# Elliotshui/ABRSimulator

Hardware: AMD Instinct MI355X
Metric: env_steps_per_sec (higher is better)
Workload: dtype f64

## Files before the change

abrsimulator_amd/_lib.py:

```python
import ctypes as C
import os
import subprocess

os.environ.setdefault("HIP_FORCE_DEV_KERNARG", "1")

import torch

_HERE = os.path.dirname(os.path.abspath(__file__))
CSRC = os.path.join(_HERE, "csrc")
DIAG_LIB_DIR = os.path.join(os.path.dirname(_HERE), "tools", "diag", "lib")


def resolve(name):
    if os.sep in name or os.path.isabs(name):
        return os.path.abspath(name)
    for d in (DIAG_LIB_DIR, CSRC):
        if os.path.exists(os.path.join(d, name)):
            return os.path.join(d, name)
    return os.path.join(DIAG_LIB_DIR, name)


SO_PATH = os.path.join(CSRC, "libabr_hip.so")
if os.environ.get("ABR_HIP_LIB"):
    SO_PATH = resolve(os.environ["ABR_HIP_LIB"])
# ... 171 lines not shown
    ("abr_env_step_policy_sampled", C.c_int, [_P, C.POINTER(Policy), C.POINTER(PolicySampling), C.c_int32, _P, _P, _P,
                                              _P, _P, _P, _P, _P]),
    ("abr_env_policy_select_ac", C.c_int, [_P, C.POINTER(Policy), C.POINTER(PolicySampling), C.POINTER(PolicyValue), _P, _P,
                                           _P, _P, _P, _P]),
    ("abr_env_step_policy_ac", C.c_int, [_P, C.POINTER(Policy), C.POINTER(PolicySampling), C.POINTER(PolicyValue),
                                         C.c_int32, _P, _P, _P, _P, _P, _P, _P, _P, _P, _P]),
    ("abr_policy_mx_weights_bytes", C.c_int, [C.POINTER(PolicyMx), C.c_int32, C.POINTER(C.c_size_t)]),
    ("abr_env_policy_select_mx", C.c_int, [_P, C.POINTER(PolicyMx), C.POINTER(PolicySampling), C.POINTER(PolicyValue), _P,
                                           _P, _P, _P, _P, _P]),
    ("abr_env_step_policy_mx", C.c_int, [_P, C.POINTER(PolicyMx), C.POINTER(PolicySampling), C.POINTER(PolicyValue),
                                         C.c_int32, _P, _P, _P, _P, _P, _P, _P, _P, _P, _P]),
    ("abr_gae", C.c_int, [_P, _P, _P, _P, _P, C.c_int32, C.c_int64, C.c_float, C.c_float, _P, _P, _P]),
    ("abr_debug_chain", C.c_int, [C.c_int32, C.c_int32, _P, _P, _P, _P, C.c_int64, _P, _P, _P, _P]),
    ("abr_debug_selfcheck", C.c_int, [_P, _P, _P]),
    ("abr_debug_drain", C.c_int, [C.c_double, C.c_double, _P, _P, C.c_int64, _P, _P, _P, C.POINTER(C.c_int32), _P]),
    ("abr_mpc_objective_grid", C.c_int, [C.POINTER(MpcConfig), C.c_int32, C.c_int32, C.c_double,
                                         _P, _P, _P, _P, _P]),
]

_libs = {}


class AbrError(RuntimeError):
    pass


def build(force=False, target="libabr_hip.so"):
    subprocess.check_call(["make", "-C", CSRC, "-s"] + (["-B"] if force else []) + [target])
    return os.path.join(CSRC, target)

# ... 44 lines not shown
```

abrsimulator_amd/csrc/abr_env.hip:

```cpp
#include <hip/hip_runtime.h>

#include <climits>
#include <cmath>
#include <cstdarg>
#include <cstdio>
#include <cstdlib>
#include <cstring>
#include <new>
#include <type_traits>
#include <vector>

#include "abr_env.h"

#ifdef ABR_SPLIT_STAMPS
#include "abr_diag_stamps.h"
#else
#define ABR_STAMP(n)
#define ABR_STAMP_INIT()
#define ABR_STAMP_FLUSH()
#define ABR_WG_TIME(slot)
#define ABR_WG_WHERE(role)
#define K3_STAMP_DECL
#define K3_STAMP(n)
#define K3_STAMP_FLUSH()
// ... 50 lines not shown
    int32_t speed_rows;
    int32_t *pl_left, *play_id;
    double *pt_sum;
    const double *br_table;
    long long *sumk;
    int32_t *k, *chunk_id, *n_su, *n_rb, *n_play, *j, *tpos, *trace_id, *offset0;
    int32_t *last_action, *n_su_obs, *n_rb_obs, *episode_no;
    uint8_t *flags, *done;
    uint8_t *action_hist;
    double *bw_hist;
    double *ep_qoe_terms;
    double *var_run;
    uint32_t *selfcheck_out;
    uint64_t sentinel;
    abrx::SpeedRuleBlock speed_rule;
};
static_assert(offsetof(EnvParams, speed_rule) == ABR_RULE_KERNARG_OFFSET, "abr_lane_jump.h reads the rule at this offset");
static_assert(sizeof(EnvParams) == 880, "the parameter block: 592 bytes + 288 of the speed rule");
static_assert(sizeof(abrx::SpeedRule) == sizeof(abr_speed_rule) &&
              offsetof(abrx::SpeedRule, lat_thr) == offsetof(abr_speed_rule, lat_thr) &&
              offsetof(abrx::SpeedRule, buf_thr) == offsetof(abr_speed_rule, buf_thr) &&
              offsetof(abrx::SpeedRule, speed) == offsetof(abr_speed_rule, speed), "abr_speed_rule: one layout");

constexpr uint32_t kTagMagic = 0x57524241u;
constexpr uint32_t kLayoutRev = 1;
struct WorkspaceTag {
    uint32_t magic, abi_version, layout_rev, n_rates;
    int64_t n_lanes;
    int32_t video_length, max_ticks, n_intervals, reserved_;
    uint64_t total_bytes;
    double chunk_length, interval, speed;
    uint8_t pad_[256 - 72];
};
static_assert(sizeof(WorkspaceTag) == 256, "the tag is one 256-byte block");
static_assert(sizeof(abrx::EpisodeSampler) == sizeof(abr_episode_sampler) &&
              offsetof(abrx::EpisodeSampler, pool) == offsetof(abr_episode_sampler, pool) &&
              offsetof(abrx::EpisodeSampler, n_pool) == offsetof(abr_episode_sampler, n_pool) &&
              offsetof(abrx::EpisodeSampler, offset_span) == offsetof(abr_episode_sampler, offset_span),
              "abr_episode_sampler: one layout");
static_assert(sizeof(abrx::EpisodeLedger) == sizeof(abr_episode_ledger) &&
// ... 373 lines not shown
        if (MODE != 0) {
            for (int32_t t = step_idx; t < n_total; t++) {
                const int64_t o = (int64_t)t * p.n_lanes + i;
                if (reward_out) reward_out[o] = 0.0f;
                if (done_out) done_out[o] = done;
                if ((MODE == 2 || MODE == 4) && actions_out) actions_out[o] = -1;
                if (obs_out)
                    write_obs(s, p, i, obs_out + (int64_t)t * ABR_OBS_DIM * p.n_lanes, last_bw);
            }
        }
    }
}

using abrx::LaneJ;

__device__ inline abrx::Tables make_tables(const EnvParams &p, bool cascade = true) {
    abrx::Tables t;
    t.G = p.G; t.interval_tick = p.interval_tick; t.avail_tick = p.avail_tick;
    t.L = p.chunk_length; t.sd = p.sd; t.max_buffer = p.max_buffer;
    t.start_up_length = p.start_up_length; t.V = p.video_length; t.max_ticks = p.max_ticks;
    t.per_lane_speed = p.lane_speeds != nullptr;
    t.speed_rows = p.lane_speeds ? p.speed_rows : 0;
    t.speed_stride = p.n_lanes; t.speeds = p.lane_speeds;
    t.drain = p.drain;
    if (p.lane_speeds || !cascade) t.drain.n = 0;
#ifdef ABR_NO_DRAIN_CASCADE
    t.drain.n = 0;
#endif
    return t;
}

__device__ inline void lanej_load(LaneJ &s, const EnvParams &p, int64_t i) {
    s.buf = p.buf[i]; s.sumk = p.sumk[i];
    s.k = p.k[i]; s.chunk_id = p.chunk_id[i]; s.n_su = p.n_su[i]; s.n_rb = p.n_rb[i];
    s.n_play = p.n_play[i]; s.cur.j = p.j[i]; s.cur.tpos = p.tpos[i];
    s.last_action = p.last_action[i];
    const uint8_t f = p.flags[i];
    s.su = f & kFlagStartUp; s.be = f & kFlagBufEmpty; s.bf = f & kFlagBufFull;
    const int32_t c = s.chunk_id < p.video_length ? s.chunk_id : p.video_length;
    s.avail_k = p.avail_tick[c];
    if (p.lane_speeds) { s.sd = p.sd_lane[i]; s.pt = p.pt_lane[i]; } else { s.sd = p.sd; s.pt = 0.0; }
    s.lane = i; s.pl_left = 0; s.play_id = 0; s.pt_sum = 0.0;
    if (p.lane_speeds && p.speed_rows >= 2) { s.pl_left = p.pl_left[i]; s.play_id = p.play_id[i]; s.pt_sum = p.pt_sum[i]; }
// ... 45 lines not shown

#ifndef ABR_JUMP_WAVES
#define ABR_JUMP_WAVES 5
#endif
#define ABR_JUMP_BOUNDS(MODE, SAMPLE) __launch_bounds__(64, ((MODE) == 1 || (MODE) == 4 || (SAMPLE) ? 4 : ABR_JUMP_WAVES))
template <int MODE, bool SAMPLE = false, bool LEDGER = false>
__global__ ABR_JUMP_BOUNDS(MODE, SAMPLE || LEDGER) void env_jump_kernel(
    EnvParams p, const int32_t *__restrict__ actions, const int32_t *__restrict__ trace_id_in,
    const int32_t *__restrict__ offset_in, const uint8_t *__restrict__ lane_mask,
    float *__restrict__ obs_out, float *__restrict__ reward_out, uint8_t *__restrict__ done_out,
    int32_t *__restrict__ actions_out, int32_t n_steps, uint64_t seed, abrx::RuleParams rule,
    abrx::EpisodeSampler smp, abrx::EpisodeLedger led) {
    const int64_t i = (int64_t)blockIdx.x * 64 + threadIdx.x;
    const bool in_range = i < p.n_lanes;
    const int32_t n_total = (MODE >= 2) ? n_steps : 1;
    const abrx::Tables tb = make_tables(p);
    LaneJ s;
    bool active = in_range, touched = in_range;
    uint8_t done = 0;
    int32_t n_su_obs = 0, n_rb_obs = 0, episode_no = 0, offset0 = 0;
    double last_bw = 0.0, hist_n = 0.0, hist_s = 0.0, var_run = 0.0;
    double g_su_obs = 0.0, g_rb_obs = 0.0;

    if (in_range) {
        if (MODE == 0) {
            if (lane_mask && !lane_mask[i]) { active = false; touched = false; }
            if (active) {
                int32_t t;
                if constexpr (SAMPLE) {
                    sampled_episode(p, smp, i, (p.flags[i] & kFlagArmed) ? p.episode_no[i] + 1 : 0, t, offset0);
                } else {
// ... 183 lines not shown
    out[ABR_F64_CHUNK_ID * n + i] = (double)p.chunk_id[i];
    out[ABR_F64_PLAY_ID * n + i] = sched ? (double)p.play_id[i] : (double)(p.n_play[i] / P);
    out[ABR_F64_LAST_BITRATE * n + i] = (double)p.last_action[i];
    out[ABR_F64_FLAGS * n + i] = (double)p.flags[i];
    out[ABR_F64_HIST_N * n + i] = p.hist_n[i];
    out[ABR_F64_HIST_SUM_INV * n + i] = p.hist_s[i];
    out[ABR_F64_TICK * n + i] = (double)p.k[i];
    out[ABR_F64_DOWNLOAD_TIME * n + i] = 0.0;
}

static size_t align_up(size_t x, size_t a) { return (x + a - 1) / a * a; }
static size_t mpc_scratch_bytes_max(size_t n_lanes) {
    return n_lanes * ((size_t)ABR_MAX_HORIZON * sizeof(double) + 2 * sizeof(int32_t));
}

struct Layout {
    size_t G, GP, interval_tick, avail_tick;
    size_t f64_state, i64_state, i32_state, u8_state, action_hist, bw_hist, ep_terms;
    size_t mpc_action, mpc_scratch;
    size_t tag;
    size_t total;
    int32_t max_ticks, n_intervals;
};

static double min_episode_ticks(const abr_env_config *c) {
    return ((double)c->video_length + 1.0) * ceil(c->chunk_length / kDt);
}
static double default_max_ticks(const abr_env_config *c) {
    double per_chunk = ceil(c->chunk_length / kDt);
    double mt = 32.0 * c->video_length * per_chunk;
    if (mt > 16.0e6) mt = 16.0e6;
    if (mt < 2.0 * min_episode_ticks(c)) mt = 2.0 * min_episode_ticks(c);
// ... 30 lines not shown
        return fail(ABR_E_INVALID, "max_ticks %g is below (video_length + 1) * ceil(chunk_length / dt) = %g: "
                    "every lane would end in ABR_DONE_TIMEOUT", mtd, min_episode_ticks(c));
    const int32_t mt = (int32_t)mtd;
    double n_iv = (double)mt * kDt / c->interval + 4.0;
    if (n_iv > 32.0e6)
        return fail(ABR_E_UNSUPPORTED, "interval %g s needs a %g-entry tick table", c->interval, n_iv);
    L->max_ticks = mt;
    L->n_intervals = (int32_t)n_iv;
    size_t o = 0;
    const size_t A = 256;
    size_t N = (size_t)n_lanes, V = (size_t)c->video_length;
    L->G = o; o = align_up(o + sizeof(double) * ((size_t)mt + 2), A);
    L->GP = o; o = align_up(o + sizeof(double) * ((size_t)mt + 2), A);
    L->interval_tick = o; o = align_up(o + sizeof(int32_t) * ((size_t)L->n_intervals + 8), A);
    L->avail_tick = o; o = align_up(o + sizeof(int32_t) * (V + 2), A);
    L->f64_state = o; o = align_up(o + sizeof(double) * 8 * N, A);
    L->i64_state = o; o = align_up(o + sizeof(long long) * 1 * N, A);
    L->i32_state = o; o = align_up(o + sizeof(int32_t) * 15 * N, A);
    L->u8_state = o; o = align_up(o + 2 * N, A);
    L->action_hist = o; o = align_up(o + V * N, A);
    L->bw_hist = o; o = align_up(o + sizeof(double) * V * N, A);
    L->ep_terms = o; o = align_up(o + sizeof(double) * 4 * N, A);
    L->mpc_action = o; o = align_up(o + sizeof(int32_t) * N, A);
    L->mpc_scratch = o; o = align_up(o + mpc_scratch_bytes_max(N), A);
    L->tag = o; o = align_up(o + sizeof(WorkspaceTag), A);
    L->total = o;
    return ABR_OK;
}

extern "C" int abr_env_workspace_bytes(const abr_env_config *cfg, int64_t n_lanes,
// ... 42 lines not shown
    EnvParams &p = e->p;
    p.n_rates = cfg->n_rates; p.video_length = cfg->video_length; p.max_ticks = mt;
    p.auto_reset = cfg->auto_reset; p.play_ticks_per_chunk = P; p.n_intervals = L.n_intervals;
    p.t_block = t_block; p.n_traces = n_traces;
    p.chunk_length = cfg->chunk_length; p.max_buffer = cfg->max_buffer;
    p.start_up_length = cfg->start_up_length;
    p.wr = cfg->rebuffer_weight; p.wv = cfg->variance_weight; p.ws = cfg->startup_weight;
    p.wl = cfg->latency_weight; p.sd = sd;
    for (int r = 0; r < ABR_MAX_RATES; r++) p.ladder[r] = cfg->ladder[r];
    p.n_lanes = n_lanes; p.lane_id_base = 0;
    char *w = (char *)workspace_dev;
    p.G = (const double *)(w + L.G); p.GP = (const double *)(w + L.GP);
    p.interval_tick = (const int32_t *)(w + L.interval_tick);
    p.avail_tick = (const int32_t *)(w + L.avail_tick);
    p.drain = abrx::make_drain_tab(sd, cfg->max_buffer + cfg->chunk_length);
    p.traces = traces_dev; p.trace_off = trace_off_dev; p.trace_len = trace_len_dev;
    const size_t N = (size_t)n_lanes;
    double *f = (double *)(w + L.f64_state);
    p.buf = f; p.last_bw = f + N; p.hist_n = f + 2 * N; p.hist_s = f + 3 * N;
    p.sd_lane = f + 4 * N; p.pt_lane = f + 5 * N; p.pt_sum = f + 6 * N; p.var_run = f + 7 * N; p.lane_speeds = nullptr;
    p.speed_rows = 1;
    p.speed_rule = abrx::SpeedRuleBlock{};
    p.sumk = (long long *)(w + L.i64_state);
    int32_t *q = (int32_t *)(w + L.i32_state);
    p.k = q; p.chunk_id = q + N; p.n_su = q + 2 * N; p.n_rb = q + 3 * N; p.n_play = q + 4 * N;
    p.j = q + 5 * N; p.tpos = q + 6 * N; p.trace_id = q + 7 * N; p.offset0 = q + 8 * N;
    p.last_action = q + 9 * N; p.n_su_obs = q + 10 * N; p.n_rb_obs = q + 11 * N;
    p.episode_no = q + 12 * N; p.pl_left = q + 13 * N; p.play_id = q + 14 * N;
    uint8_t *u = (uint8_t *)(w + L.u8_state);
    p.flags = u; p.done = u + N;
    p.action_hist = (uint8_t *)(w + L.action_hist);
    p.bw_hist = (double *)(w + L.bw_hist);
    p.ep_qoe_terms = (double *)(w + L.ep_terms);
    e->mpc_action = (int32_t *)(w + L.mpc_action);
    e->mpc_scratch = (void *)(w + L.mpc_scratch);

    hipStream_t st = (hipStream_t)stream;
    hipError_t he;
#define UP(dst, vec)                                                                           \
    he = hipMemcpyAsync((void *)(dst), (vec).data(), (vec).size() * sizeof((vec)[0]),          \
                        hipMemcpyHostToDevice, st);                                            \
    if (he != hipSuccess) { delete e; return fail(ABR_E_HIP, "table upload: %s", hipGetErrorString(he)); }
    UP(p.G, G) UP(p.GP, GP) UP(p.interval_tick, itick) UP(p.avail_tick, atick)
#undef UP
    he = hipMemsetAsync(w + L.f64_state, 0, L.total - L.f64_state, st);
    if (he == hipSuccess) he = hipMemsetAsync(p.done, ABR_DONE_EPISODE, N, st);
    {
        WorkspaceTag &tg = e->tag;
        memset(&tg, 0, sizeof(tg));
        tg.magic = kTagMagic; tg.abi_version = ABR_ABI_VERSION; tg.layout_rev = kLayoutRev; tg.n_rates = (uint32_t)cfg->n_rates;
        tg.n_lanes = n_lanes; tg.video_length = cfg->video_length; tg.max_ticks = mt; tg.n_intervals = L.n_intervals;
        tg.total_bytes = L.total; tg.chunk_length = cfg->chunk_length; tg.interval = cfg->interval; tg.speed = cfg->speed;
        e->tag_dev = w + L.tag;
        if (he == hipSuccess) he = hipMemcpyAsync(e->tag_dev, &tg, sizeof(tg), hipMemcpyHostToDevice, st);
    }
    if (he == hipSuccess) he = hipStreamSynchronize(st);
    if (he != hipSuccess) { delete e; return fail(ABR_E_HIP, "workspace init: %s", hipGetErrorString(he)); }
    *env_out = e;
// ... 2272 lines not shown

extern "C" int abr_debug_drain(double sd, double max_level, const double *x0_dev, const int32_t *n_dev, int64_t count,
                               double *x_out_dev, int32_t *a_out_dev, uint8_t *hit_out_dev, int32_t *stages_out,
                               void *stream) {
    if (!x0_dev || !n_dev || !x_out_dev || !a_out_dev || !hit_out_dev) return fail(ABR_E_INVALID, "NULL device pointer");
    if (count < 1) return fail(ABR_E_INVALID, "count must be >= 1");
    const abrx::DrainTab tab = abrx::make_drain_tab(sd, max_level);
    if (stages_out) *stages_out = tab.n;
    if (tab.n == 0) return fail(ABR_E_UNSUPPORTED, "no cascade for sd %g below %g: the kernels use the general chains", sd, max_level);
    hipLaunchKernelGGL(drain_debug_kernel, dim3((unsigned)((count + 63) / 64)), dim3(64), 0, (hipStream_t)stream, tab, sd,
                       x0_dev, n_dev, count, x_out_dev, a_out_dev, hit_out_dev);
    HIP_TRY(hipGetLastError());
    return ABR_OK;
}

__global__ void mpc_grid_kernel(int B, int H, int V, double L, double max_buffer, double wv,
                                double wr, int chunk, int prev, double buffer,
                                const double *__restrict__ pred, const double *__restrict__ br,
                                const double *__restrict__ sz, double *__restrict__ J_out,
                                int64_t total) {
    const int64_t f = (int64_t)blockIdx.x * blockDim.x + threadIdx.x;
    if (f >= total) return;
    int R[ABR_MAX_HORIZON + 1];
    {
        int64_t t = f;
        for (int i = H; i >= 1; i--) { R[i] = (int)(t % B); t /= B; }
        R[0] = prev < 0 ? prev + B : prev;
    }
    double q = 0.0, v = 0.0, rb = 0.0, buf = buffer;
    for (int i = 0; i < H; i++) {
// ... 44 lines not shown
```

abrsimulator_amd/csrc/abr_env_roles.h:

```cpp
#ifndef ABR_ENV_ROLES_H
#define ABR_ENV_ROLES_H


#ifndef ABR_SPLIT3_CASCADE
#define ABR_SPLIT3_CASCADE 0
#endif
#ifndef ABR_PRIO_D
#define ABR_PRIO_D 2
#endif
#ifndef ABR_PRIO_P
#define ABR_PRIO_P 1
#endif
#ifndef ABR_PRIO_S
#define ABR_PRIO_S 0
#endif

struct SplitMail {
    double dl[2][64];
    int32_t n_dl[2][64], k_start[2][64], step[2][64], action[2][64], avail_next[2][64], flags[2][64];
    int32_t fb_step[2][64], fb_k[2][64], fb_chunk[2][64], fb_episode[2][64], fb_alive[2][64];
    double fb_buf[2][64];
    int32_t fb_pf[2][64];
    int32_t any_alive[2];
};
// ... 273 lines not shown
    v.episode_no = 0; v.b_step = 0; v.b_alive = false; v.was_done = true;
}

__device__ __forceinline__ void role_p3_begin(PVars &v, const EnvParams &p) {
    const int64_t i = (int64_t)blockIdx.x * 64 + (threadIdx.x & 63);
    player_clear(v, p);
    if (i < p.n_lanes) {
        v.was_done = p.done[i] != 0;
        lanej_load(v.s, p, i);
        v.episode_no = p.episode_no[i];
        v.b_alive = !v.was_done;
    }
    ABR_STAMP_INIT();
}

template <int MODE, class M2>
__device__ __forceinline__ void role_p3_pre(PVars &v, const EnvParams &p, SplitMail &m, M2 &m2,
                                            int32_t n_total, int32_t t, int cb2) {
    const int l = threadIdx.x & 63;
    const int cb = t & 1, pb = (t + 1) & 1;
    const abrx::Tables tb = make_tables(p, ABR_SPLIT3_CASCADE != 0);
    const bool speeds = p.lane_speeds != nullptr;
    LaneJ &s = v.s;
    int32_t meta = 0;
    ABR_STAMP(8);
    if (v.b_alive && v.b_step < n_total && t >= 1) {
        int32_t fl = m.flags[pb][l];
        int32_t r_step = m.step[pb][l], r_k = m.k_start[pb][l], r_a = m.action[pb][l], r_ndl = m.n_dl[pb][l],
                r_avail = m.avail_next[pb][l];
        double r_dl = m.dl[pb][l];
        asm volatile("" : "+v"(fl), "+v"(r_step), "+v"(r_k), "+v"(r_a), "+v"(r_ndl), "+v"(r_avail), "+v"(r_dl));
        if ((fl & kRecValid) && r_step == v.b_step && r_k == s.k) {
            const int32_t a = r_a;
            meta = kS3Valid | (a & 0xff);
            m2.step[cb2][l] = v.b_step;
            if (fl & kRecBadAct) {
                meta |= kS3Bad;
                v.b_alive = false;
            } else {
                abrx::Download d;
                d.dl = r_dl; d.n_dl = r_ndl; d.hit = (fl & kRecHit) != 0;
                const abrx::StepResult sr = abrx::lanej_after_download(s, tb, d, r_avail, a);
                if (sr.hit) meta |= kS3Hit;
                if (sr.ended) meta |= kS3Ended;
                if (sr.timeout) meta |= kS3Timeout;
                m2.dl[cb2][l] = d.dl; m2.n_dl[cb2][l] = d.n_dl;
                m2.nrb_r[cb2][l] = s.n_rb; m2.nsu_r[cb2][l] = s.n_su;
                if (sr.ended || sr.timeout) {
                    m2.lat[cb2][l] = player_latency(p, s);
                    if (p.auto_reset && sr.ended) {
                        abrx::lanej_init_player(s, tb);
                        v.episode_no++;
                        meta |= kS3Reset;
                        if (!abrx::lanej_wait_call(s, tb)) { meta |= kS3Timeout2; v.b_alive = false; }
                    } else v.b_alive = false;
                }
                m2.buf[cb2][l] = s.buf; m2.k[cb2][l] = s.k; m2.nplay_o[cb2][l] = s.n_play;
// ... 247 lines not shown
        service_write_obs(v, p, i, obs_out ? obs_out + (int64_t)t2 * ABR_OBS_DIM * p.n_lanes : nullptr);
    }
}

template <int MODE, bool SAMPLE = false, bool LEDGER = false>
__global__ __launch_bounds__(192) __attribute__((amdgpu_waves_per_eu(1, 3))) void env_split3_kernel(
    EnvParams p, const int32_t *__restrict__ actions, float *__restrict__ obs_out,
    float *__restrict__ reward_out, uint8_t *__restrict__ done_out,
    int32_t *__restrict__ actions_out, int32_t n_steps, uint64_t seed, abrx::EpisodeSampler smp,
    abrx::EpisodeLedger led) {
    (void)led;
    __shared__ SplitMail m;
    __shared__ SplitMail2 m2;
    __shared__ ActRing ring;
    const int32_t n_total = (MODE >= 2) ? n_steps : 1;
    const int role = __builtin_amdgcn_readfirstlane((int)(threadIdx.x >> 6));
    if constexpr (MODE == 9) { selfcheck_answer(p); return; }
#ifdef ABR_SPLIT_STAMPS
    if (fresh_params().n_lanes != p.n_lanes || fresh_params().traces != p.traces) __builtin_trap();
#endif
    __shared__ RolePark3 park;
    DVars dv;
    role_d_begin(dv, p);
    if (role == 0) ABR_WG_TIME(0);
    ABR_WG_WHERE(role);
    if (role == 0) __builtin_amdgcn_s_setprio(ABR_PRIO_D);
    else if (role == 1) { __builtin_amdgcn_s_setprio(ABR_PRIO_P); PVars v; role_p3_begin(v, p); p_park(park.p, v); }
    else { __builtin_amdgcn_s_setprio(ABR_PRIO_S); SVars v; role_s_begin(v, p, ring); s_park(park.s, v); }
    for (int32_t t = 0;; t++) {
        if (role == 0) {
            if (t > 0) role_d_validate<SAMPLE>(dv, m, make_tables(p, ABR_SPLIT3_CASCADE != 0), t - 1);
            role_d_pre<MODE, true, SAMPLE>(dv, p, m, &ring, actions, actions_out, n_total, seed, t, smp);
        } else if (role == 1) {
            PVars v; p_unpark(park.p, v, p);
            role_p3_pre<MODE>(v, p, m, m2, n_total, t, t & 1);
            p_park(park.p, v);
        } else {
            SVars v; s_unpark(park.s, v);
            role_s_pre<MODE, SAMPLE, LEDGER>(v, p, m, m2, ring, obs_out, reward_out, done_out, n_total, seed, t);
            s_park(park.s, v);
        }
        __syncthreads();
        ABR_STAMP(role == 0 ? 5 : (role == 1 ? 18 : 22));
        if (!m.any_alive[t & 1]) break;
    }
    if (role == 0) { role_d_end(dv, p); ABR_WG_TIME(1); }
    else if (role == 1) { PVars v; p_unpark(park.p, v, p); role_p3_end(v, p); ABR_WG_TIME(2); }
    else { SVars v; s_unpark(park.s, v); role_s_end<MODE, SAMPLE, LEDGER>(v, p, m2, obs_out, reward_out, done_out, actions_out, n_total, smp); ABR_WG_TIME(3); }
}

// ... 35 lines not shown
        v.last_bw = p.last_bw[i]; v.hist_n = p.hist_n[i]; v.hist_s = p.hist_s[i]; v.var_run = p.var_run[i];
        v.g_su_obs = p.G[v.n_su_obs]; v.g_rb_obs = p.G[v.n_rb_obs];
        v.pv.b_alive = !v.done;
    }
    ABR_STAMP_INIT();
}

template <int MODE, bool SAMPLE = false, bool LEDGER = false>
__device__ __forceinline__ void role_p2_pre(P2Vars &v, const EnvParams &, SplitMail &m, float *__restrict__ obs_out,
                                            float *__restrict__ reward_out, uint8_t *__restrict__ done_out,
                                            int32_t n_total, int32_t t) {
    const EnvParams &p = fresh_params();
    const int l = threadIdx.x & 63;
    const int64_t i = (int64_t)blockIdx.x * 64 + l;
    const int cb = t & 1, pb = (t + 1) & 1;
    const abrx::Tables tb = make_tables(p);
    LaneJ &s = v.pv.s;
    ABR_STAMP(8);
    if (v.pv.b_alive && v.pv.b_step < n_total && t >= 1) {
        const int32_t fl = m.flags[pb][l];
        const int32_t r_step = m.step[pb][l], r_k = m.k_start[pb][l], r_a = m.action[pb][l], r_ndl = m.n_dl[pb][l],
                      r_avail = m.avail_next[pb][l];
        const double r_dl = m.dl[pb][l];
        if ((fl & kRecValid) && r_step == v.pv.b_step && r_k == s.k) {
            const int64_t o = (int64_t)v.pv.b_step * p.n_lanes + i;
            float *obs = obs_out ? obs_out + (int64_t)v.pv.b_step * ABR_OBS_DIM * p.n_lanes : nullptr;
            const int32_t a = r_a;
            if (fl & kRecBadAct) {
                v.done |= ABR_DONE_BADACT;
                if (reward_out) ABR_OUT(reward_out[o], 0.0f);
                if (done_out) ABR_OUT(done_out[o], (uint8_t)v.done);
// ... 93 lines not shown
    (void)led;
    __shared__ SplitMail m;
    const int32_t n_total = (MODE >= 2) ? n_steps : 1;
    const int role = __builtin_amdgcn_readfirstlane((int)(threadIdx.x >> 6));
    if constexpr (MODE == 9) { selfcheck_answer(p); return; }
#ifdef ABR_SPLIT_STAMPS
    if (fresh_params().n_lanes != p.n_lanes || fresh_params().traces != p.traces) __builtin_trap();
#endif
    __shared__ RolePark2 park;
    DVars dv;
    role_d_begin(dv, p);
    if (role == 0) __builtin_amdgcn_s_setprio(2);
    else { P2Vars v; role_p2_begin(v, p); p2_park(park.p, v); }
    for (int32_t t = 0;; t++) {
        if (role == 0) {
            if (t > 0) role_d_validate<SAMPLE>(dv, m, make_tables(p), t - 1);
            role_d_pre<MODE, false, SAMPLE>(dv, p, m, nullptr, actions, actions_out, n_total, seed, t, smp);
        } else {
            P2Vars v; p2_unpark(park.p, v, fresh_params());
            role_p2_pre<MODE, SAMPLE, LEDGER>(v, p, m, obs_out, reward_out, done_out, n_total, t);
            p2_park(park.p, v);
        }
        __syncthreads();
        ABR_STAMP(role == 0 ? 5 : 18);
        if (!m.any_alive[t & 1]) break;
    }
    if (role == 0) role_d_end(dv, p);
    else { P2Vars v; p2_unpark(park.p, v, fresh_params()); role_p2_end<MODE, SAMPLE>(v, p, obs_out, reward_out, done_out, actions_out, n_total, smp); }
}

#endif
// ... 1 lines not shown
```

abrsimulator_amd/csrc/abr_exact_jump.h:

```cpp
#ifndef ABR_EXACT_JUMP_H
#define ABR_EXACT_JUMP_H

#include <stdint.h>
#include <string.h>

#if defined(__HIPCC__)
#define ABR_HD __host__ __device__ inline
#else
#define ABR_HD inline
#endif

namespace abrx {

ABR_HD int expo(double x) {
    uint64_t b;
#if defined(__HIP_DEVICE_COMPILE__)
    b = (uint64_t)__double_as_longlong(x);
#else
    memcpy(&b, &x, 8);
#endif
    return (int)((b >> 52) & 0x7ff);
}

ABR_HD double pow2_biased(int e) {
// ... 255 lines not shown
    }
#if defined(__HIP_DEVICE_COMPILE__)
#pragma unroll 1
#endif
#ifdef ABR_CASCADE_HOOK
    const int32_t a_stages = a;
#endif
    while (a < m && x > 0.0) { x = x - sd; a++; }
#ifdef ABR_CASCADE_HOOK
    ABR_CASCADE_HOOK(tb_e_hi, tb_n, x_io, x, a_stages, a - a_stages, m);
#endif
    x_io = x; a_out = a;
    return a > 0 && x <= 0.0;
}

}
#endif
```

abrsimulator_amd/csrc/abr_lane_jump.h:

```cpp
#ifndef ABR_LANE_JUMP_H
#define ABR_LANE_JUMP_H

#include <math.h>

#include "abr_exact_jump.h"

#ifndef ABR_STAMP
#define ABR_STAMP(n)
#endif

namespace abrx {

constexpr double kTickDt = 0.01;
#ifndef ABR_K_DRAIN_TAIL
#define ABR_K_DRAIN_TAIL 16
#endif
constexpr int kPrologue = 16;
#ifndef ABR_PCHUNKS
#define ABR_PCHUNKS 12
#endif
#ifndef ABR_PCHECK
#define ABR_PCHECK 0x892
#endif
constexpr int kPChunks = ABR_PCHUNKS;
// ... 20 lines not shown
    int32_t log_rows, reserved_;
};

struct Tables {
    const double *G;
    const int32_t *interval_tick;
    const int32_t *avail_tick;
    double L, sd, max_buffer, start_up_length;
    int32_t V, max_ticks;
    bool per_lane_speed;
    int32_t speed_rows;
    int64_t speed_stride;
    const double *speeds;
    const SpeedRuleBlock *rule = nullptr;
    DrainTab drain;
};

struct Cursor {
    int32_t j;
    int32_t tpos;
    int32_t tlen;
    const double *trace;
};

struct LaneJ {
    double buf;
    double sd;
    double pt;
    long long sumk;
    int32_t k, chunk_id, n_su, n_rb, n_play, avail_k, last_action;
// ... 21 lines not shown

ABR_HD void lanej_init(LaneJ &s, const Tables &t, int32_t offset0) {
    lanej_init_player(s, t);
    cursor_init(s.cur, offset0);
}

ABR_HD void lanej_play(LaneJ &s, const Tables &t, int32_t a) {
    if (!t.per_lane_speed || a <= 0) return;
    int32_t done = 0;
    double x = s.pt;
    chain<STOP_GE>(x, s.sd, 1.0e300, a, done);
    s.pt = x;
}

constexpr int kDrainTail = ABR_K_DRAIN_TAIL;
ABR_HD bool drain_to_zero(double &b_io, double sd, int32_t m, int32_t &a_out) {
    ChainState cs;
    cs.x = b_io; cs.eb = -1;
    const double tail = (double)kDrainTail * sd;
    int32_t a = 0;
    bool below = false;
    while (a < m && !below) a += chain_segment<STOP_LE>(cs, -sd, tail, m - a, below);
    double b = cs.x;
    ABR_STAMP(24);
#ifdef ABR_DRAIN_HOOK
    const int32_t a_seg = a;
#endif
#if defined(__HIP_DEVICE_COMPILE__)
#pragma unroll 1
#endif
// ... 1 lines not shown
    ABR_STAMP(25);
#ifdef ABR_DRAIN_HOOK
    ABR_DRAIN_HOOK(a > 0 && b <= 0.0, a - a_seg);
#endif
    b_io = b; a_out = a;
    return a > 0 && b <= 0.0;
}

ABR_HD bool lanej_drain(const Tables &t, double &b_io, double sd, int32_t m, int32_t &a_out) {
    if (t.drain.n > 0 && !wave_any(!(b_io < t.drain.top))) {
        const bool zero = drain_cascade(t.drain, sd, b_io, m, a_out);
        ABR_STAMP(24);
        return zero;
    }
    return drain_to_zero(b_io, sd, m, a_out);
}

ABR_HD void sched_begin_chunk(LaneJ &s, const Tables &t, int32_t k, double b) {
    double v;
    if (t.speed_rows == kSpeedRowsRule) {
#if defined(__HIP_DEVICE_COMPILE__) && defined(ABR_RULE_KERNARG_OFFSET)
        auto kp = __builtin_amdgcn_kernarg_segment_ptr();
        asm volatile("" : "+s"(kp));
        const SpeedRuleBlock &rb = *(const SpeedRuleBlock *)((const char *)kp + ABR_RULE_KERNARG_OFFSET);
#else
        const SpeedRuleBlock &rb = *t.rule;
#endif
        v = speed_rule_eval(rb.rule, t.G[k] - s.pt, b);
        if (s.play_id < rb.log_rows) rb.log[(int64_t)s.play_id * t.speed_stride + s.lane] = v;
    } else {
// ... 23 lines not shown
    int32_t a_tot = 0;
    bool hit = false;
    while (a_tot < m && !hit) {
        if (s.pl_left == 0) sched_begin_chunk(s, t, s.k + a_tot, b);
        const int32_t run = (m - a_tot < s.pl_left) ? m - a_tot : s.pl_left;
        int32_t a = 0;
        if (STOP == STOP_LE) hit = drain_to_zero(b, s.sd, run, a);
        else hit = chain<STOP_LT>(b, -s.sd, thr, run, a);
        sched_played(s, t, a);
        a_tot += a;
    }
    a_out = a_tot;
    return hit;
}

ABR_HD void lanej_idle(LaneJ &s, const Tables &t, int32_t m) {
    if (m <= 0) return;
    if (s.su && s.buf >= t.start_up_length) s.su = false;
    ABR_STAMP(23);
    if (s.su) {
        s.n_su += m;
    } else if (s.be) {
        s.n_rb += m;
    } else {
        int32_t a = 0;
        double b = s.buf;
        bool zero;
        if (t.speed_rows >= 2) zero = sched_drain<STOP_LE>(s, t, b, 0.0, m, a);
        else { zero = lanej_drain(t, b, s.sd, m, a); lanej_play(s, t, a); }
        s.n_play += a;
        s.sumk += (long long)a * s.k + ((long long)a * (a - 1)) / 2;
        if (zero) { b = 0.0; s.be = true; s.n_rb += (m - a + 1); }
        s.buf = b;
        s.bf = b >= t.max_buffer;
    }
    s.k += m;
}

ABR_HD bool lanej_wait_call(LaneJ &s, const Tables &t) {
    const int32_t mt = t.max_ticks;
    if (s.k >= s.avail_k && !s.bf) return true;
    int32_t w = s.avail_k - s.k;
    if (w < 0) w = 0;
    if (w > mt - s.k) w = mt - s.k;
    lanej_idle(s, t, w);
    if (s.k >= mt) return false;
    if (s.bf) {
        if (s.su || s.be) {
            if (s.su) s.n_su += mt - s.k; else s.n_rb += mt - s.k;
            s.k = mt;
            return false;
        }
        int32_t a = 0;
        double b = s.buf;
        bool cleared;
        if (t.speed_rows >= 2) cleared = sched_drain<STOP_LT>(s, t, b, t.max_buffer, mt - s.k, a);
        else { cleared = chain<STOP_LT>(b, -s.sd, t.max_buffer, mt - s.k, a); lanej_play(s, t, a); }
        s.n_play += a;
        s.sumk += (long long)a * s.k + ((long long)a * (a - 1)) / 2;
        s.k += a;
// ... 150 lines not shown
        ke = adv ? (ke_next < mt ? ke_next : mt) : ke;
        s.j += adv ? 1 : 0;
        s.tpos = adv ? tn : s.tpos;
        cs.eb = adv ? -1 : cs.eb;
        tn = (s.tpos + 1 == s.tlen) ? 0 : s.tpos + 1;
        bw_next = s.trace[(uint32_t)tn];
        ke_next = t.interval_tick[(uint32_t)(s.j + 2)];
        kk += chain_segment<STOP_GE>(cs, c, target, ke - kk, hit);
    }
    Download d;
    d.dl = cs.x; d.n_dl = kk - k; d.hit = hit;
    return d;
}

ABR_HD StepResult lanej_after_download(LaneJ &s, const Tables &t, const Download &d,
                                       int32_t avail_next, int32_t action) {
    StepResult r;
    r.bw = 0.0; r.hit = false; r.ended = false; r.timeout = false;
    const int32_t mt = t.max_ticks;
    const bool hit = d.hit;
    const int32_t n_dl = d.n_dl;
    const double g_ndl = t.G[n_dl];
    lanej_idle(s, t, hit ? n_dl - 1 : n_dl);
    ABR_STAMP(10);
    if (!hit) { r.timeout = true; return r; }
    const bool playing = !(s.be || s.su);
    double b = s.buf + t.L;
    if (playing) {
        s.sumk += s.k; s.n_play++;
        if (t.speed_rows >= 2) {
            if (s.pl_left == 0) sched_begin_chunk(s, t, s.k, b);
            b = b - s.sd;
            sched_played(s, t, 1);
        } else { b = b - s.sd; lanej_play(s, t, 1); }
    }
    s.bf = b >= t.max_buffer;
    s.be = b <= 0.0;
    if (s.be) b = 0.0;
// ... 13 lines not shown
        s.n_rb += (!s.su && s.be) ? 1 : 0;
        r.timeout = !lanej_wait_call(s, t);
    }
    ABR_STAMP(12);
    return r;
}

ABR_HD bool lanej_gate_possible(double buf, bool su, bool be, int32_t n_dl, const Tables &t) {
    return !su && !be && !t.per_lane_speed && (buf + t.L) - (double)n_dl * t.sd >= t.max_buffer - 1.0e-6;
}
ABR_HD bool lanej_predict_next_call(double buf, int32_t k, int32_t n_dl, int32_t avail_next, const Tables &t,
                                    int32_t &k_next, double *buf_next = nullptr) {
    const int32_t mt = t.max_ticks;
    double b = buf;
    int32_t a = 0;
    if (n_dl > 1 && lanej_drain(t, b, t.sd, n_dl - 1, a)) return false;
    b = b + t.L;
    b = b - t.sd;
    if (b <= 0.0) return false;
    bool bf = b >= t.max_buffer;
    k += n_dl;
    if (k >= mt) return false;
    if (!(k >= avail_next && !bf)) {
        int32_t w = avail_next - k;
        if (w < 0) w = 0;
        if (w > mt - k) w = mt - k;
        if (w > 0) {
            if (lanej_drain(t, b, t.sd, w, a)) return false;
            bf = b >= t.max_buffer;
            k += w;
        }
        if (k >= mt) return false;
        if (bf) {
            a = 0;
            if (!chain<STOP_LT>(b, -t.sd, t.max_buffer, mt - k, a)) return false;
            k += a;
            if (b <= 0.0) return false;
        }
    }
    k_next = k;
    if (buf_next) *buf_next = b;
    return true;
}
// ... 554 lines not shown
```

include/abr_env.h:

```cpp
#ifndef ABR_ENV_H
#define ABR_ENV_H

#include <stddef.h>
#include <stdint.h>

#ifdef __cplusplus
extern "C" {
#endif

#define ABR_ABI_VERSION 4
#define ABR_MAX_RATES 16
#define ABR_MAX_HORIZON 8

#define ABR_OK 0
#define ABR_E_INVALID (-1)
#define ABR_E_WORKSPACE (-2)
#define ABR_E_HIP (-3)
#define ABR_E_UNSUPPORTED (-4)

#define ABR_DONE_EPISODE 0x1
#define ABR_DONE_TIMEOUT 0x2
#define ABR_DONE_BADACT 0x4
#define ABR_DONE_BADARG 0x8

// ... 330 lines not shown
int abr_gae(const float *reward_dev, const float *values_dev, const float *last_value_dev, const uint8_t *done_dev,
            const int32_t *actions_dev, int32_t n_steps, int64_t n_lanes, float gamma, float lam, float *adv_out_dev,
            float *ret_out_dev, void *stream);

int abr_mpc_objective_grid(const abr_mpc_config *cfg, int32_t chunk, int32_t prev_bitrate,
                           double buffer_level, const double *pred_dev, const double *br_table_dev,
                           const double *sz_table_dev, double *J_out_dev, void *stream);

int abr_debug_chain(int32_t stop_kind, int32_t estimate_bias, const double *x0_dev,
                    const double *c_dev, const double *thr_dev, const int32_t *n_dev, int64_t count,
                    double *x_out_dev, int32_t *a_out_dev, uint8_t *hit_out_dev, void *stream);

int abr_debug_drain(double sd, double max_level, const double *x0_dev, const int32_t *n_dev, int64_t count,
                    double *x_out_dev, int32_t *a_out_dev, uint8_t *hit_out_dev, int32_t *stages_out, void *stream);

int abr_debug_selfcheck(abr_env *env, uint32_t *result_dev, void *stream);

#ifdef __cplusplus
}
#endif
#endif
```

Baseline: 12.39 billion.

## Add precomputed run-dry table and wave-uniform drain for buffer depletion

Builds a host-side table of exact floating-point thresholds at which repeated subtraction of the drain rate runs the buffer dry, uploads it into the workspace, and adds a new drain path that probes a four-entry window to decide in closed form whether a lane empties within the step budget. Lanes that go dry skip the iterative per-exponent drain loop, and the remaining lanes use a wave-uniform stage loop. This aims to cut divergent sequential drain iterations in the idle/after-download path, at the cost of an extra table load per step, a larger kernel parameter block and workspace, and more code complexity. A debug entry point is added to check the new drain against the old one.

```diff
diff --git a/abrsimulator_amd/_lib.py b/abrsimulator_amd/_lib.py
--- a/abrsimulator_amd/_lib.py
+++ b/abrsimulator_amd/_lib.py
@@ -209,6 +209,7 @@
     ("abr_debug_chain", C.c_int, [C.c_int32, C.c_int32, _P, _P, _P, _P, C.c_int64, _P, _P, _P, _P]),
     ("abr_debug_selfcheck", C.c_int, [_P, _P, _P]),
     ("abr_debug_drain", C.c_int, [C.c_double, C.c_double, _P, _P, C.c_int64, _P, _P, _P, C.POINTER(C.c_int32), _P]),
+    ("abr_debug_drain_lanes", C.c_int, [C.c_double, C.c_double, _P, _P, C.c_int64, _P, _P, _P, C.POINTER(C.c_int32), _P]),
     ("abr_mpc_objective_grid", C.c_int, [C.POINTER(MpcConfig), C.c_int32, C.c_int32, C.c_double,
                                          _P, _P, _P, _P, _P]),
 ]
diff --git a/abrsimulator_amd/csrc/abr_env.hip b/abrsimulator_amd/csrc/abr_env.hip
--- a/abrsimulator_amd/csrc/abr_env.hip
+++ b/abrsimulator_amd/csrc/abr_env.hip
@@ -88,16 +88,18 @@
     uint32_t *selfcheck_out;
     uint64_t sentinel;
     abrx::SpeedRuleBlock speed_rule;
+    const double *dry_tab;
+    int32_t dry_n, reserved_dry_;
 };
 static_assert(offsetof(EnvParams, speed_rule) == ABR_RULE_KERNARG_OFFSET, "abr_lane_jump.h reads the rule at this offset");
-static_assert(sizeof(EnvParams) == 880, "the parameter block: 592 bytes + 288 of the speed rule");
+static_assert(sizeof(EnvParams) == 896, "the parameter block: 592 bytes + 288 of the speed rule + 16 of the run-dry table");
 static_assert(sizeof(abrx::SpeedRule) == sizeof(abr_speed_rule) &&
               offsetof(abrx::SpeedRule, lat_thr) == offsetof(abr_speed_rule, lat_thr) &&
               offsetof(abrx::SpeedRule, buf_thr) == offsetof(abr_speed_rule, buf_thr) &&
               offsetof(abrx::SpeedRule, speed) == offsetof(abr_speed_rule, speed), "abr_speed_rule: one layout");
 
 constexpr uint32_t kTagMagic = 0x57524241u;
-constexpr uint32_t kLayoutRev = 1;
+constexpr uint32_t kLayoutRev = 2;
 struct WorkspaceTag {
     uint32_t magic, abi_version, layout_rev, n_rates;
     int64_t n_lanes;
@@ -501,7 +503,18 @@
 
 using abrx::LaneJ;
 
-__device__ inline abrx::Tables make_tables(const EnvParams &p, bool cascade = true) {
+constexpr int kDrainsChains = 0, kDrainsCascade = 1, kDrainsLanes = 2;
+#ifndef ABR_SPLIT3_DRAINS
+#define ABR_SPLIT3_DRAINS (ABR_SPLIT3_CASCADE ? 1 : 0)
+#endif
+#ifndef ABR_SPLIT_DRAINS
+#define ABR_SPLIT_DRAINS 1
+#endif
+#ifndef ABR_JUMP_DRAINS
+#define ABR_JUMP_DRAINS 1
+#endif
+__device__ inline abrx::Tables make_tables(const EnvParams &p, int drains = kDrainsCascade) {
+    const bool cascade = drains != kDrainsChains;
     abrx::Tables t;
     t.G = p.G; t.interval_tick = p.interval_tick; t.avail_tick = p.avail_tick;
     t.L = p.chunk_length; t.sd = p.sd; t.max_buffer = p.max_buffer;
@@ -514,6 +527,8 @@
 #ifdef ABR_NO_DRAIN_CASCADE
     t.drain.n = 0;
 #endif
+    t.dry = p.dry_tab;
+    t.dry_n = (drains == kDrainsLanes && t.drain.n > 0) ? p.dry_n : 0;
     return t;
 }
 
@@ -589,7 +604,7 @@
     const int64_t i = (int64_t)blockIdx.x * 64 + threadIdx.x;
     const bool in_range = i < p.n_lanes;
     const int32_t n_total = (MODE >= 2) ? n_steps : 1;
-    const abrx::Tables tb = make_tables(p);
+    const abrx::Tables tb = make_tables(p, ABR_JUMP_DRAINS);
     LaneJ s;
     bool active = in_range, touched = in_range;
     uint8_t done = 0;
@@ -803,8 +818,10 @@
     return n_lanes * ((size_t)ABR_MAX_HORIZON * sizeof(double) + 2 * sizeof(int32_t));
 }
 
+constexpr int32_t kDryCap = 8192;
+
 struct Layout {
-    size_t G, GP, interval_tick, avail_tick;
+    size_t G, GP, interval_tick, avail_tick, dry_tab;
     size_t f64_state, i64_state, i32_state, u8_state, action_hist, bw_hist, ep_terms;
     size_t mpc_action, mpc_scratch;
     size_t tag;
@@ -865,6 +882,7 @@
     L->GP = o; o = align_up(o + sizeof(double) * ((size_t)mt + 2), A);
     L->interval_tick = o; o = align_up(o + sizeof(int32_t) * ((size_t)L->n_intervals + 8), A);
     L->avail_tick = o; o = align_up(o + sizeof(int32_t) * (V + 2), A);
+    L->dry_tab = o; o = align_up(o + sizeof(double) * (size_t)kDryCap, A);
     L->f64_state = o; o = align_up(o + sizeof(double) * 8 * N, A);
     L->i64_state = o; o = align_up(o + sizeof(long long) * 1 * N, A);
     L->i32_state = o; o = align_up(o + sizeof(int32_t) * 15 * N, A);
@@ -937,6 +955,9 @@
     p.interval_tick = (const int32_t *)(w + L.interval_tick);
     p.avail_tick = (const int32_t *)(w + L.avail_tick);
     p.drain = abrx::make_drain_tab(sd, cfg->max_buffer + cfg->chunk_length);
+    std::vector<double> dry((size_t)kDryCap, 0.0);
+    p.dry_tab = (const double *)(w + L.dry_tab);
+    p.dry_n = abrx::make_dry_tab(sd, cfg->max_buffer + cfg->chunk_length, dry.data(), kDryCap);
     p.traces = traces_dev; p.trace_off = trace_off_dev; p.trace_len = trace_len_dev;
     const size_t N = (size_t)n_lanes;
     double *f = (double *)(w + L.f64_state);
@@ -964,7 +985,7 @@
     he = hipMemcpyAsync((void *)(dst), (vec).data(), (vec).size() * sizeof((vec)[0]),          \
                         hipMemcpyHostToDevice, st);                                            \
     if (he != hipSuccess) { delete e; return fail(ABR_E_HIP, "table upload: %s", hipGetErrorString(he)); }
-    UP(p.G, G) UP(p.GP, GP) UP(p.interval_tick, itick) UP(p.avail_tick, atick)
+    UP(p.G, G) UP(p.GP, GP) UP(p.interval_tick, itick) UP(p.avail_tick, atick) UP(p.dry_tab, dry)
 #undef UP
     he = hipMemsetAsync(w + L.f64_state, 0, L.total - L.f64_state, st);
     if (he == hipSuccess) he = hipMemsetAsync(p.done, ABR_DONE_EPISODE, N, st);
@@ -3267,6 +3288,49 @@
     return ABR_OK;
 }
 
+__global__ void drain_lanes_debug_kernel(abrx::DrainTab tab, const double *__restrict__ dry, int32_t dry_n, double sd,
+                                         const double *__restrict__ x0, const int32_t *__restrict__ n, int64_t count,
+                                         double *__restrict__ x_out, int32_t *__restrict__ a_out,
+                                         uint8_t *__restrict__ hit_out) {
+    const int64_t i = (int64_t)blockIdx.x * blockDim.x + threadIdx.x;
+    if (i >= count) return;
+    abrx::Tables t;
+    t.G = nullptr; t.interval_tick = nullptr; t.avail_tick = nullptr;
+    t.L = 0.0; t.sd = sd; t.max_buffer = 0.0; t.start_up_length = 0.0; t.V = 0; t.max_ticks = 0;
+    t.per_lane_speed = false; t.speed_rows = 0; t.speed_stride = 0; t.speeds = nullptr;
+    t.drain = tab; t.dry = dry; t.dry_n = dry_n;
+    double x = x0[i];
+    int32_t a = 0;
+    const bool zero = abrx::lanej_drain_level(t, x, sd, n[i], a);
+    x_out[i] = x; a_out[i] = a; hit_out[i] = zero ? 1 : 0;
+}
+
+extern "C" int abr_debug_drain_lanes(double sd, double max_level, const double *x0_dev, const int32_t *n_dev, int64_t count,
+                                     double *x_out_dev, int32_t *a_out_dev, uint8_t *hit_out_dev, int32_t *stages_out,
+                                     void *stream) {
+    if (!x0_dev || !n_dev || !x_out_dev || !a_out_dev || !hit_out_dev) return fail(ABR_E_INVALID, "NULL device pointer");
+    if (count < 1) return fail(ABR_E_INVALID, "count must be >= 1");
+    const abrx::DrainTab tab = abrx::make_drain_tab(sd, max_level);
+    if (stages_out) *stages_out = tab.n;
+    std::vector<double> dry((size_t)kDryCap, 0.0);
+    const int32_t dry_n = abrx::make_dry_tab(sd, max_level, dry.data(), kDryCap);
+    if (tab.n == 0 || dry_n == 0)
+        return fail(ABR_E_UNSUPPORTED, "no run-dry table for sd %g below %g: the kernels keep their other drains", sd, max_level);
+    hipStream_t st = (hipStream_t)stream;
+    double *dry_dev = nullptr;
+    HIP_TRY(hipMalloc((void **)&dry_dev, sizeof(double) * (size_t)dry_n));
+    hipError_t he = hipMemcpyAsync(dry_dev, dry.data(), sizeof(double) * (size_t)dry_n, hipMemcpyHostToDevice, st);
+    if (he == hipSuccess) {
+        hipLaunchKernelGGL(drain_lanes_debug_kernel, dim3((unsigned)((count + 63) / 64)), dim3(64), 0, st, tab, dry_dev, dry_n,
+                           sd, x0_dev, n_dev, count, x_out_dev, a_out_dev, hit_out_dev);
+        he = hipGetLastError();
+    }
+    if (he == hipSuccess) he = hipStreamSynchronize(st);
+    (void)hipFree(dry_dev);
+    if (he != hipSuccess) return fail(ABR_E_HIP, "abr_debug_drain_lanes: %s", hipGetErrorString(he));
+    return ABR_OK;
+}
+
 __global__ void mpc_grid_kernel(int B, int H, int V, double L, double max_buffer, double wv,
                                 double wr, int chunk, int prev, double buffer,
                                 const double *__restrict__ pred, const double *__restrict__ br,
diff --git a/abrsimulator_amd/csrc/abr_env_roles.h b/abrsimulator_amd/csrc/abr_env_roles.h
--- a/abrsimulator_amd/csrc/abr_env_roles.h
+++ b/abrsimulator_amd/csrc/abr_env_roles.h
@@ -311,16 +311,19 @@
     ABR_STAMP_INIT();
 }
 
-template <int MODE, class M2>
+template <int MODE, int DRAINS = ABR_SPLIT3_DRAINS, class M2>
 __device__ __forceinline__ void role_p3_pre(PVars &v, const EnvParams &p, SplitMail &m, M2 &m2,
                                             int32_t n_total, int32_t t, int cb2) {
     const int l = threadIdx.x & 63;
     const int cb = t & 1, pb = (t + 1) & 1;
-    const abrx::Tables tb = make_tables(p, ABR_SPLIT3_CASCADE != 0);
+    const abrx::Tables tb = make_tables(p, DRAINS);
     const bool speeds = p.lane_speeds != nullptr;
     LaneJ &s = v.s;
     int32_t meta = 0;
     ABR_STAMP(8);
+    abrx::DryWin dw;
+    dw.j = 0; dw.w0 = dw.w1 = dw.w2 = dw.w3 = 1.0e308;
+    if (tb.dry_n > 0) dw = abrx::dry_probe(tb.dry, tb.dry_n, tb.drain.rcp, s.buf);
     if (v.b_alive && v.b_step < n_total && t >= 1) {
         int32_t fl = m.flags[pb][l];
         int32_t r_step = m.step[pb][l], r_k = m.k_start[pb][l], r_a = m.action[pb][l], r_ndl = m.n_dl[pb][l],
@@ -337,7 +340,7 @@
             } else {
                 abrx::Download d;
                 d.dl = r_dl; d.n_dl = r_ndl; d.hit = (fl & kRecHit) != 0;
-                const abrx::StepResult sr = abrx::lanej_after_download(s, tb, d, r_avail, a);
+                const abrx::StepResult sr = abrx::lanej_after_download(s, tb, d, r_avail, a, &dw);
                 if (sr.hit) meta |= kS3Hit;
                 if (sr.ended) meta |= kS3Ended;
                 if (sr.timeout) meta |= kS3Timeout;
@@ -615,6 +618,7 @@
     __shared__ SplitMail2 m2;
     __shared__ ActRing ring;
     const int32_t n_total = (MODE >= 2) ? n_steps : 1;
+    constexpr int DRAINS = SAMPLE ? (ABR_SPLIT3_CASCADE ? 1 : 0) : ABR_SPLIT3_DRAINS;
     const int role = __builtin_amdgcn_readfirstlane((int)(threadIdx.x >> 6));
     if constexpr (MODE == 9) { selfcheck_answer(p); return; }
 #ifdef ABR_SPLIT_STAMPS
@@ -630,11 +634,11 @@
     else { __builtin_amdgcn_s_setprio(ABR_PRIO_S); SVars v; role_s_begin(v, p, ring); s_park(park.s, v); }
     for (int32_t t = 0;; t++) {
         if (role == 0) {
-            if (t > 0) role_d_validate<SAMPLE>(dv, m, make_tables(p, ABR_SPLIT3_CASCADE != 0), t - 1);
+            if (t > 0) role_d_validate<SAMPLE>(dv, m, make_tables(p, DRAINS), t - 1);
             role_d_pre<MODE, true, SAMPLE>(dv, p, m, &ring, actions, actions_out, n_total, seed, t, smp);
         } else if (role == 1) {
             PVars v; p_unpark(park.p, v, p);
-            role_p3_pre<MODE>(v, p, m, m2, n_total, t, t & 1);
+            role_p3_pre<MODE, DRAINS>(v, p, m, m2, n_total, t, t & 1);
             p_park(park.p, v);
         } else {
             SVars v; s_unpark(park.s, v);
@@ -700,7 +704,7 @@
     const int l = threadIdx.x & 63;
     const int64_t i = (int64_t)blockIdx.x * 64 + l;
     const int cb = t & 1, pb = (t + 1) & 1;
-    const abrx::Tables tb = make_tables(p);
+    const abrx::Tables tb = make_tables(p, ABR_SPLIT_DRAINS);
     LaneJ &s = v.pv.s;
     ABR_STAMP(8);
     if (v.pv.b_alive && v.pv.b_step < n_total && t >= 1) {
@@ -824,7 +828,7 @@
     else { P2Vars v; role_p2_begin(v, p); p2_park(park.p, v); }
     for (int32_t t = 0;; t++) {
         if (role == 0) {
-            if (t > 0) role_d_validate<SAMPLE>(dv, m, make_tables(p), t - 1);
+            if (t > 0) role_d_validate<SAMPLE>(dv, m, make_tables(p, ABR_SPLIT_DRAINS), t - 1);
             role_d_pre<MODE, false, SAMPLE>(dv, p, m, nullptr, actions, actions_out, n_total, seed, t, smp);
         } else {
             P2Vars v; p2_unpark(park.p, v, fresh_params());
diff --git a/abrsimulator_amd/csrc/abr_exact_jump.h b/abrsimulator_amd/csrc/abr_exact_jump.h
--- a/abrsimulator_amd/csrc/abr_exact_jump.h
+++ b/abrsimulator_amd/csrc/abr_exact_jump.h
@@ -1,6 +1,7 @@
 #ifndef ABR_EXACT_JUMP_H
 #define ABR_EXACT_JUMP_H
 
+#include <math.h>
 #include <stdint.h>
 #include <string.h>
 
@@ -293,5 +294,98 @@
     return a > 0 && x <= 0.0;
 }
 
-}
-#endif
+struct DryWin {
+    double w0, w1, w2, w3;
+    int32_t j;
+};
+
+inline int32_t make_dry_tab(double sd, double max_level, double *out, int32_t cap) {
+    if (make_drain_tab(sd, max_level).n == 0 || !out) return 0;
+    double t = 4.9406564584124654e-324;
+    int32_t n = 0;
+    for (;;) {
+        if (n >= cap) return 0;
+        out[n++] = t;
+        if (t > max_level) break;
+        double c = t + sd;
+        for (;;) {
+            const double d = nextafter(c, -1.0);
+            if (d > 0.0 && d - sd >= t) c = d; else break;
+        }
+        while (!(c - sd >= t)) c = nextafter(c, 1.0e308);
+        t = c;
+    }
+    return n >= 4 ? n : 0;
+}
+
+ABR_HD DryWin dry_probe(const double *__restrict__ T, int32_t tn, double rcp, double x) {
+    DryWin w;
+    const int32_t j = (int32_t)clamp0(sat_i32(x * rcp) - 1, tn - 4);
+    w.j = j;
+    w.w0 = T[j]; w.w1 = T[j + 1]; w.w2 = T[j + 2]; w.w3 = T[j + 3];
+    return w;
+}
+
+ABR_HD bool drain_lanes(const DrainTab &tb_in, const DryWin &w, double sd, double &x_io, int32_t m, int32_t &a_out) {
+    int32_t e_lo = tb_in.e_hi - tb_in.n + 1, e_hi = tb_in.e_hi;
+    double tb_rcp = tb_in.rcp;
+#if defined(__HIP_DEVICE_COMPILE__)
+    asm volatile("" : "+v"(sd), "+v"(tb_rcp), "+v"(e_lo), "+v"(e_hi));
+    e_lo = __builtin_amdgcn_readfirstlane(e_lo);
+#endif
+    double x = x_io;
+    const int32_t cnt = (x >= w.w0 ? 1 : 0) + (x >= w.w1 ? 1 : 0) + (x >= w.w2 ? 1 : 0) + (x >= w.w3 ? 1 : 0);
+    const int32_t N = w.j + cnt;
+    const bool dry = (cnt >= 1) & (cnt <= 3) & (N <= m);
+    const int32_t lim = dry ? 0 : m;
+    int32_t a = 0;
+    int32_t e = expo(x);
+    e = e < e_hi ? e : e_hi;
+#ifdef ABR_LANES_HOOK
+    int32_t passes = 0;
+#endif
+#if defined(__HIP_DEVICE_COMPILE__)
+#pragma unroll 1
+#endif
+    while (wave_any((a < lim) & (e >= e_lo))) {
+        const int ec = e > e_lo ? e : e_lo;
+        const double base = pow2_biased(ec);
+        const double u = pow2_biased(ec - 52);
+        const double S = (base + sd) - base;
+        const double T = (S >= sd) ? S : S + u;
+        const double B = base + T;
+        const double g = x - B;
+        int32_t q = sat_i32(g * tb_rcp);
+        const double r = g - (double)q * S;
+        q -= (r < 0.0) ? 1 : 0;
+        q += (r >= S) ? 1 : 0;
+        int32_t n = q + 1;
+        const int32_t left = lim - a;
+        n = n < left ? n : left;
+        n = (e >= e_lo) ? n : 0;
+        n = n > 0 ? n : 0;
+        x = x - (double)n * S;
+        a += n;
+        e -= 1;
+#ifdef ABR_LANES_HOOK
+        passes++;
+#endif
+    }
+#ifdef ABR_LANES_HOOK
+    const int32_t a_stages = a;
+#endif
+#if defined(__HIP_DEVICE_COMPILE__)
+#pragma unroll 1
+#endif
+    while (a < lim && x > 0.0) { x = x - sd; a++; }
+#ifdef ABR_LANES_HOOK
+    ABR_LANES_HOOK(passes, a - a_stages, dry, m);
+#endif
+    const bool zero = dry | (a > 0 && x <= 0.0);
+    x_io = zero ? 0.0 : x;
+    a_out = dry ? N : a;
+    return zero;
+}
+
+}
+#endif
diff --git a/abrsimulator_amd/csrc/abr_lane_jump.h b/abrsimulator_amd/csrc/abr_lane_jump.h
--- a/abrsimulator_amd/csrc/abr_lane_jump.h
+++ b/abrsimulator_amd/csrc/abr_lane_jump.h
@@ -58,6 +58,8 @@
     const double *speeds;
     const SpeedRuleBlock *rule = nullptr;
     DrainTab drain;
+    const double *dry = nullptr;
+    int32_t dry_n = 0;
 };
 
 struct Cursor {
@@ -109,6 +111,9 @@
 }
 
 constexpr int kDrainTail = ABR_K_DRAIN_TAIL;
+#ifndef ABR_DRY_TEST_WAIT
+#define ABR_DRY_TEST_WAIT 0
+#endif
 ABR_HD bool drain_to_zero(double &b_io, double sd, int32_t m, int32_t &a_out) {
     ChainState cs;
     cs.x = b_io; cs.eb = -1;
@@ -140,6 +145,27 @@
         return zero;
     }
     return drain_to_zero(b_io, sd, m, a_out);
+}
+
+template <bool DRY_TEST = true>
+ABR_HD bool lanej_drain_level(const Tables &t, double &b_io, double sd, int32_t m, int32_t &a_out,
+                              const DryWin *pre = nullptr) {
+    if (t.dry_n > 0 && !wave_any(!(b_io < t.drain.top))) {
+        DryWin w;
+        if (!DRY_TEST) {
+            w.j = 0; w.w0 = w.w1 = w.w2 = w.w3 = 1.0e308;
+        } else if (pre) {
+            w = *pre;
+        } else {
+            w = dry_probe(t.dry, t.dry_n, t.drain.rcp, b_io);
+        }
+        const bool zero = drain_lanes(t.drain, w, sd, b_io, m, a_out);
+        ABR_STAMP(24);
+        return zero;
+    }
+    const bool zero = lanej_drain(t, b_io, sd, m, a_out);
+    if (zero) b_io = 0.0;
+    return zero;
 }
 
 ABR_HD void sched_begin_chunk(LaneJ &s, const Tables &t, int32_t k, double b) {
@@ -193,7 +219,8 @@
     return hit;
 }
 
-ABR_HD void lanej_idle(LaneJ &s, const Tables &t, int32_t m) {
+template <bool DRY_TEST = true>
+ABR_HD void lanej_idle(LaneJ &s, const Tables &t, int32_t m, const DryWin *pre = nullptr) {
     if (m <= 0) return;
     if (s.su && s.buf >= t.start_up_length) s.su = false;
     ABR_STAMP(23);
@@ -206,7 +233,7 @@
         double b = s.buf;
         bool zero;
         if (t.speed_rows >= 2) zero = sched_drain<STOP_LE>(s, t, b, 0.0, m, a);
-        else { zero = lanej_drain(t, b, s.sd, m, a); lanej_play(s, t, a); }
+        else { zero = lanej_drain_level<DRY_TEST>(t, b, s.sd, m, a, pre); lanej_play(s, t, a); }
         s.n_play += a;
         s.sumk += (long long)a * s.k + ((long long)a * (a - 1)) / 2;
         if (zero) { b = 0.0; s.be = true; s.n_rb += (m - a + 1); }
@@ -222,7 +249,7 @@
     int32_t w = s.avail_k - s.k;
     if (w < 0) w = 0;
     if (w > mt - s.k) w = mt - s.k;
-    lanej_idle(s, t, w);
+    lanej_idle<ABR_DRY_TEST_WAIT != 0>(s, t, w);
     if (s.k >= mt) return false;
     if (s.bf) {
         if (s.su || s.be) {
@@ -403,14 +430,14 @@
 }
 
 ABR_HD StepResult lanej_after_download(LaneJ &s, const Tables &t, const Download &d,
-                                       int32_t avail_next, int32_t action) {
+                                       int32_t avail_next, int32_t action, const DryWin *pre = nullptr) {
     StepResult r;
     r.bw = 0.0; r.hit = false; r.ended = false; r.timeout = false;
     const int32_t mt = t.max_ticks;
     const bool hit = d.hit;
     const int32_t n_dl = d.n_dl;
     const double g_ndl = t.G[n_dl];
-    lanej_idle(s, t, hit ? n_dl - 1 : n_dl);
+    lanej_idle(s, t, hit ? n_dl - 1 : n_dl, pre);
     ABR_STAMP(10);
     if (!hit) { r.timeout = true; return r; }
     const bool playing = !(s.be || s.su);
@@ -454,7 +481,7 @@
     const int32_t mt = t.max_ticks;
     double b = buf;
     int32_t a = 0;
-    if (n_dl > 1 && lanej_drain(t, b, t.sd, n_dl - 1, a)) return false;
+    if (n_dl > 1 && lanej_drain_level(t, b, t.sd, n_dl - 1, a)) return false;
     b = b + t.L;
     b = b - t.sd;
     if (b <= 0.0) return false;
@@ -466,7 +493,7 @@
         if (w < 0) w = 0;
         if (w > mt - k) w = mt - k;
         if (w > 0) {
-            if (lanej_drain(t, b, t.sd, w, a)) return false;
+            if (lanej_drain_level<ABR_DRY_TEST_WAIT != 0>(t, b, t.sd, w, a)) return false;
             bf = b >= t.max_buffer;
             k += w;
         }
diff --git a/include/abr_env.h b/include/abr_env.h
--- a/include/abr_env.h
+++ b/include/abr_env.h
@@ -368,6 +368,9 @@
 int abr_debug_drain(double sd, double max_level, const double *x0_dev, const int32_t *n_dev, int64_t count,
                     double *x_out_dev, int32_t *a_out_dev, uint8_t *hit_out_dev, int32_t *stages_out, void *stream);
 
+int abr_debug_drain_lanes(double sd, double max_level, const double *x0_dev, const int32_t *n_dev, int64_t count,
+                          double *x_out_dev, int32_t *a_out_dev, uint8_t *hit_out_dev, int32_t *stages_out, void *stream);
+
 int abr_debug_selfcheck(abr_env *env, uint32_t *result_dev, void *stream);
 
 #ifdef __cplusplus
```

Result: slower. 12.05 billion (-2.7%).
